# Triton-AI/Triton-Racer-Sim

Measured on AMD Instinct MI355X. Metric: env-steps/s (whole node) at N envs x 120x160 RGB, higher is better.
Workload: dtype f32 state / f64 nearest-point / u8 image; 1 GPU; 1024 envs/GPU x 1 GPU, bicycle physics + L1 nearest point + 120x160 RGB pinhole rasteriser = BASELINE configs[2], generated_track 1185 pts, synthetic controls seed 0x5EED, auto-reset; envs_total=1024, envs_per_gpu=1024, img_h=120, img_w=160, depth=False, steps_per_launch=1, step_mode=resident worker (posted steps), prewarm_steps=8400, launcher=self

## Files before the change

### triton-racer-sim_amd/csrc/trsim_post.hpp

```cpp
#pragma once

#include <algorithm>
#include <chrono>
#include <cstddef>
#include <cstdint>
#include <cstring>

#include "trsim_plan.hpp"

namespace trsim {

constexpr int kSlots = 8;

struct WEntry {
    uint64_t seq_lo;
    const float* steer; const float* thr; const float* brk;
    const uint8_t* reset;
    uint32_t synth, pad0;
    uint64_t seq;
    uint64_t pad1;
};
static_assert(sizeof(WEntry) == 64, "one entry per 64-B line");
constexpr int kTagLo = 0, kTagHi = 6;
static_assert(offsetof(WEntry, seq_lo) == 8 * kTagLo && offsetof(WEntry, seq) == 8 * kTagHi && offsetof(WEntry, reset) == 32, "tag placement");

struct Mailbox {
    alignas(64) uint64_t close;
    uint64_t posted;
    alignas(64) uint64_t exited;
    uint64_t consumed;
    uint64_t error;
    uint64_t started;
    alignas(64) uint64_t done[kSlots];
    alignas(64) WEntry ring[kSlots];
};

constexpr unsigned long long kExitNormal = 1ull, kExitNotCoresident = 2ull;
constexpr unsigned long long kCloseLeave = 1ull, kCloseCancel = 2ull;
constexpr unsigned kRetryMs0 = 100;

enum GiveUp : unsigned { kGiveUpPost = 1, kGiveUpCamRing = 2, kGiveUpPhysics = 3, kGiveUpForward = 4, kGiveUpBarrier = 5, kGiveUpInjected = 7, kGiveUpLdsBase = 9 };
constexpr const char* kGiveUpText[10] = {"", "waiting for a post", "camera ring back-pressure", "waiting for the physics team", "forwarding the last arrivals",
                                         "team barrier of the dynamic-brightness batch", "", "abort injected by trs_resident_debug_abort (test hook)", "",
                                         "dynamic LDS segment not at offset 0"};
inline const char* give_up_text(unsigned code) { return code < 10 ? kGiveUpText[code] : "?"; }

inline uint64_t host_load(const uint64_t* p) { return __atomic_load_n(p, __ATOMIC_ACQUIRE); }
inline void host_store(uint64_t* p, uint64_t v) { __atomic_store_n(p, v, __ATOMIC_RELEASE); }

struct PostLedger {
    using Clock = std::chrono::steady_clock;
    bool enabled = false;
    bool running = false;
    bool launched = false;
    bool fell_back = false;
    bool broken = false;
    uint64_t base = 0;
    uint64_t seen_done = 0;
    unsigned retry_ms = kRetryMs0;
    Clock::time_point t_fallback{};

    void restart(uint64_t step) { base = seen_done = step; }
    void absorb(uint64_t step) { launched = false; restart(step); }
    void note_launch(uint64_t step) { launched = true; restart(step); }
    void observe(uint64_t count) { seen_done = std::max(seen_done, count); }
    bool orphans(uint64_t posted, uint64_t step) const { return posted > seen_done && posted == step; }
    bool must_wait(uint64_t s) const { return s >= base + kSlots; }
    void worker_launched() { running = true; }
    void worker_ended() { running = false; }
    void worker_had_the_gpu() { retry_ms = kRetryMs0; }
    void gave_up() { broken = true; }
    void clear_fault() { broken = false; }
    void fall_back(Clock::time_point now) { enabled = false; fell_back = true; t_fallback = now; }
    bool retry_due(Clock::time_point now) const { return !enabled && fell_back && !broken && now - t_fallback >= std::chrono::milliseconds(retry_ms); }
    bool select(uint64_t step) { retry_ms = kRetryMs0; return turn_on(step); }
    bool reselect(uint64_t step) { retry_ms = std::min(retry_ms * 2u, 2000u); launched = false; return turn_on(step); }
    void deselect() { enabled = false; }
private:
// ... 33 lines not shown
```

### triton-racer-sim_amd/csrc/trsim_resident.hip

```cpp
#include <hip/hip_runtime.h>

#include <algorithm>
#include <array>
#include <atomic>
#include <chrono>
#include <cstdint>
#include <cstdlib>
#include <cstring>
#include <mutex>
#include <string>
#include <utility>

#include "../../include/trsim.h"
#include "../../include/trsim_spec.h"
#include "trsim_device.hpp"
#include "trsim_env.hpp"
#include "trsim_internal.hpp"
#include "trsim_post.hpp"

namespace trsim {

struct DevCtl {
    alignas(64) unsigned long long word;
    alignas(64) WEntry ring[kSlots];
// ... 21 lines not shown
#ifndef TRS_RESIDENT_DIAG
#define TRS_RESIDENT_DIAG 0
#endif
constexpr int kDiag = TRS_RESIDENT_DIAG;

constexpr unsigned kDefaultLifeUs = 50000;
#ifndef TRS_PHYS_PRIO_MAX_ENVS
#define TRS_PHYS_PRIO_MAX_ENVS 1
#endif

struct Resident {
    PostLedger led;
    PinnedBuf<Mailbox> mb;
    DevBuf<DevCtl> dc;
    hipStream_t sC = nullptr;
    uint64_t gen_start = 0; Variant gen_variant = 0;
    bool dc_ready = false; uint64_t dc_ready_for = 0;
    std::chrono::steady_clock::time_point t_launch{};
    unsigned idle_us = 2000;
    unsigned life_us = kDefaultLifeUs;
    PinnedBuf<> hctl;
    int lds_bytes = 0, lds_off_ctl = 0, lds_off_dyn = 0, lds_off_hill = 0;
    long long pw_capacity_envs = 0;
    int pw_capacity_lds = -1;
};

}

namespace {

using namespace trsim;
using u64 = unsigned long long;

constexpr u64 kExitBit = 1ull << 63, kAbortBit = 1ull << 62, kCountMask = kAbortBit - 1;
constexpr int kFellBack = trsim::kResidentFellBack;

constexpr int kMaxDevices = 64;
struct DeviceSlot { std::recursive_mutex mu; trs_env* owner = nullptr; };
DeviceSlot g_dev[kMaxDevices];
struct DevLock {
    std::unique_lock<std::recursive_mutex> lk;
    explicit DevLock(const trs_env* e) : lk(g_dev[(unsigned)e->device % kMaxDevices].mu) {}
};
inline DeviceSlot& slot_of(const trs_env* e) { return g_dev[(unsigned)e->device % kMaxDevices]; }

__device__ __forceinline__ u64 sys_load64(const void* p) { return __hip_atomic_load((const u64*)p, __ATOMIC_RELAXED, __HIP_MEMORY_SCOPE_SYSTEM); }
__device__ __forceinline__ unsigned sys_load32(const void* p) { return __hip_atomic_load((const unsigned*)p, __ATOMIC_RELAXED, __HIP_MEMORY_SCOPE_SYSTEM); }
__device__ __forceinline__ void sys_store64(void* p, u64 v) { __hip_atomic_store((u64*)p, v, __ATOMIC_RELAXED, __HIP_MEMORY_SCOPE_SYSTEM); }
__device__ __forceinline__ u64 agent_load64(const void* p) { return __hip_atomic_load((const u64*)p, __ATOMIC_RELAXED, __HIP_MEMORY_SCOPE_AGENT); }
__device__ __forceinline__ void agent_store64(void* p, u64 v) { __hip_atomic_store((u64*)p, v, __ATOMIC_RELAXED, __HIP_MEMORY_SCOPE_AGENT); }
__device__ __forceinline__ u64 lds_load64(const u64* p) { return __hip_atomic_load(p, __ATOMIC_RELAXED, __HIP_MEMORY_SCOPE_WORKGROUP); }
__device__ __forceinline__ void lds_store64(u64* p, u64 v) { __hip_atomic_store(p, v, __ATOMIC_RELAXED, __HIP_MEMORY_SCOPE_WORKGROUP); }
__device__ __forceinline__ int lds_load32(const int* p) { return __hip_atomic_load(p, __ATOMIC_RELAXED, __HIP_MEMORY_SCOPE_WORKGROUP); }
__device__ __forceinline__ void lds_store32(int* p, int v) { __hip_atomic_store(p, v, __ATOMIC_RELAXED, __HIP_MEMORY_SCOPE_WORKGROUP); }
__device__ __forceinline__ void drain_vmem() { asm volatile("s_waitcnt vmcnt(0)" ::: "memory"); }
__device__ __forceinline__ void drain_lds() { asm volatile("s_waitcnt lgkmcnt(0)" ::: "memory"); }

__device__ __forceinline__ void wait_vmcnt_le(int n)
{
    switch (__builtin_amdgcn_readfirstlane(n < 0 ? 0 : (n > 63 ? 63 : n))) {
#define W(i) case i: asm volatile("s_waitcnt vmcnt(" #i ")" ::: "memory"); break;
    W(0) W(1) W(2) W(3) W(4) W(5) W(6) W(7) W(8) W(9) W(10) W(11) W(12) W(13) W(14) W(15) W(16) W(17) W(18) W(19) W(20) W(21) W(22) W(23) W(24) W(25) W(26) W(27) W(28) W(29) W(30) W(31) W(32) W(33) W(34) W(35) W(36) W(37) W(38) W(39) W(40) W(41) W(42) W(43) W(44) W(45) W(46) W(47) W(48) W(49) W(50) W(51) W(52) W(53) W(54) W(55) W(56) W(57) W(58) W(59) W(60) W(61) W(62) W(63)
#undef W
    }
}

template <typename T>
__device__ __forceinline__ T sys_load_val(const T* p)
{
    return __hip_atomic_load((const __attribute__((address_space(1))) T*)(uintptr_t)p, __ATOMIC_RELAXED, __HIP_MEMORY_SCOPE_SYSTEM);
}

struct WLds {
    u64* word;
    u64* fwd;
    int* arrive;
    int* pprog;
    int* rread;
    float* slot;
    float* lst;
};

__device__ __forceinline__ WLds wlds_of(unsigned char* base, int epw)
{
    WLds l;
    l.word = reinterpret_cast<u64*>(base);
    l.fwd = reinterpret_cast<u64*>(base + 8);
    l.arrive = reinterpret_cast<int*>(base + 16);
    l.pprog = reinterpret_cast<int*>(base + 64);
    l.rread = l.pprog + epw;
    l.slot = reinterpret_cast<float*>(base + wlds_slot_off(epw));
    l.lst = l.slot + (size_t)kCamDepth * epw * kSlotWords;
    return l;
}

__device__ __forceinline__ void worker_abort(const WParams& wp, const WLds& l, unsigned code)
{
    sys_store64(&wp.mb->error, ((u64)code << 32) | (u64)blockIdx.x);
    __hip_atomic_fetch_or(&wp.dc->word, kAbortBit, __ATOMIC_RELAXED, __HIP_MEMORY_SCOPE_AGENT);
    __hip_atomic_fetch_or(l.word, kAbortBit, __ATOMIC_RELAXED, __HIP_MEMORY_SCOPE_WORKGROUP);
}

struct Leader { u64 known, t_last, t_start; };

__device__ __forceinline__ u64 lane_u64(u64 v, int k)
{
    return ((u64)(unsigned)__builtin_amdgcn_readlane((int)(v >> 32), k) << 32) | (u64)(unsigned)__builtin_amdgcn_readlane((int)v, k);
}

__device__ __forceinline__ int dispatcher_take(const WParams& wp, const WLds& l, Leader& L, int lane, bool& close_req)
{
    const u64 v = sys_load64(reinterpret_cast<const u64*>(&wp.mb->ring[0]) + lane);
    const u64 c = sys_load64(&wp.mb->close);
    close_req = c != 0ull;
    int fresh = 0;
    for (; fresh < kSlots; ++fresh) {
        const int slot = (int)((L.known + (u64)fresh) & (kSlots - 1));
        const int hi = slot * 8 + kTagHi, lo = slot * 8 + kTagLo;
        const u64 tag = ((u64)(unsigned)__shfl((int)(v >> 32), hi, 64) << 32) | (u64)(unsigned)__shfl((int)v, hi, 64);
        const u64 tag_lo = ((u64)(unsigned)__shfl((int)(v >> 32), lo, 64) << 32) | (u64)(unsigned)__shfl((int)v, lo, 64);
        if (tag != L.known + (u64)fresh + 1 || tag_lo != tag) break;
    }
    if (fresh == 0) return 0;
    const int rel = (int)(((u64)(lane >> 3) - L.known) & (kSlots - 1));
    if (rel < fresh) agent_store64(reinterpret_cast<u64*>(&wp.dc->ring[0]) + lane, v);
    drain_vmem();
    L.known += (u64)fresh;
    if (lane == 0) {
        __hip_atomic_fetch_max(&wp.dc->word, L.known, __ATOMIC_RELAXED, __HIP_MEMORY_SCOPE_AGENT);
        __hip_atomic_fetch_max(l.word, L.known, __ATOMIC_RELAXED, __HIP_MEMORY_SCOPE_WORKGROUP);
    }
    return fresh;
}

__device__ __forceinline__ void dispatcher_publish_exit(const WParams& wp, const WLds& l, u64 count, int lane)
{
    if (lane == 0) {
        const u64 w = count | kExitBit;
        const u64 old_g = __hip_atomic_fetch_max(&wp.dc->word, w, __ATOMIC_RELAXED, __HIP_MEMORY_SCOPE_AGENT);
        if (old_g & kAbortBit) __hip_atomic_fetch_or(&wp.dc->word, kAbortBit, __ATOMIC_RELAXED, __HIP_MEMORY_SCOPE_AGENT);
        const u64 old_l = __hip_atomic_fetch_max(l.word, w, __ATOMIC_RELAXED, __HIP_MEMORY_SCOPE_WORKGROUP);
        if ((old_l | old_g) & kAbortBit) __hip_atomic_fetch_or(l.word, kAbortBit, __ATOMIC_RELAXED, __HIP_MEMORY_SCOPE_WORKGROUP);
    }
    drain_vmem();
}

__device__ __forceinline__ void worker_checkin(const WParams& wp)
{
    __hip_atomic_fetch_add(&wp.dc->checkin[0], 1u, __ATOMIC_RELAXED, __HIP_MEMORY_SCOPE_AGENT);
}

constexpr unsigned kGo = 1u, kNoGo = 2u;

__device__ __forceinline__ unsigned decision_load(const WParams& wp) { return __hip_atomic_load(&wp.dc->decision[0], __ATOMIC_RELAXED, __HIP_MEMORY_SCOPE_AGENT); }

__device__ __forceinline__ unsigned decision_close(const WParams& wp, unsigned want, int lane, bool& won)
{
    unsigned seen = 0u;
    if (lane == 0) {
        unsigned expected = 0u;
        const bool ok = __hip_atomic_compare_exchange_strong(&wp.dc->decision[0], &expected, want, __ATOMIC_RELAXED, __ATOMIC_RELAXED, __HIP_MEMORY_SCOPE_AGENT);
        seen = ok ? (want | 0x100u) : expected;
    }
    seen = (unsigned)__builtin_amdgcn_readfirstlane((int)seen);
    won = (seen & 0x100u) != 0u;
    return seen & 0xffu;
}

__device__ __forceinline__ void leave_not_coresident(const WParams& wp, const WLds& l, int lane, bool won)
{
    if (won) {
        if (lane == 0) sys_store64(&wp.mb->consumed, wp.start);
        drain_vmem();
        if (lane == 0) sys_store64(&wp.mb->exited, kExitNotCoresident);
    }
    dispatcher_publish_exit(wp, l, wp.start, lane);
}

__device__ __forceinline__ int dispatcher_checkin(const WParams& wp, const WLds& l, int lane)
{
    const u64 t0 = (u64)wall_clock64();
    bool cancel = sys_load64(&wp.mb->close) == kCloseCancel, won = false;
    for (unsigned spins = 0; !cancel; ++spins) {
        if (decision_load(wp) == kNoGo) { leave_not_coresident(wp, l, lane, false); return 0; }
        if (__hip_atomic_load(&wp.dc->checkin[0], __ATOMIC_RELAXED, __HIP_MEMORY_SCOPE_AGENT) >= (unsigned)wp.n_blocks) {
            if (decision_close(wp, kGo, lane, won) != kGo) { leave_not_coresident(wp, l, lane, false); return 0; }
            if (lane == 0) sys_store64(&wp.mb->started, 1ull);
            return 1;
        }
        if (agent_load64(&wp.dc->word) & kAbortBit) {
            if (lane == 0) __hip_atomic_fetch_or(l.word, kAbortBit, __ATOMIC_RELAXED, __HIP_MEMORY_SCOPE_WORKGROUP);
            return 0;
        }
        if ((u64)wall_clock64() - t0 > wp.checkin_ticks) break;
        if ((spins & 63u) == 63u) cancel = sys_load64(&wp.mb->close) == kCloseCancel;
        __builtin_amdgcn_s_sleep(4);
    }
    const unsigned d = decision_close(wp, kNoGo, lane, won);
    if (d == kGo) { if (lane == 0) sys_store64(&wp.mb->started, 1ull); return 1; }
    leave_not_coresident(wp, l, lane, won);
    return 0;
}

__device__ __forceinline__ int leader_wait_decision(const WParams& wp, const WLds& l, int lane)
{
    const u64 t0 = (u64)wall_clock64();
    for (;;) {
        unsigned d = decision_load(wp);
        if (d == 0u && (u64)wall_clock64() - t0 > 2ull * wp.checkin_ticks) {
            bool won = false;
            d = decision_close(wp, kNoGo, lane, won);
            if (d == kNoGo) { leave_not_coresident(wp, l, lane, won); return 0; }
        }
        if (d == kGo) return 1;
        if (d == kNoGo) { leave_not_coresident(wp, l, lane, false); return 0; }
        if (agent_load64(&wp.dc->word) & kAbortBit) {
            if (lane == 0) __hip_atomic_fetch_or(l.word, kAbortBit, __ATOMIC_RELAXED, __HIP_MEMORY_SCOPE_WORKGROUP);
            return 0;
        }
        __builtin_amdgcn_s_sleep(8);
    }
}

__device__ __forceinline__ void dispatcher_run(const WParams& wp, const WLds& l, int lane)
{
    if (!dispatcher_checkin(wp, l, lane)) return;
    Leader L{wp.start, (u64)wall_clock64(), (u64)wall_clock64()};
    for (;;) {
        if ((lds_load64(l.word) | agent_load64(&wp.dc->word)) & kAbortBit) {
            if (lane == 0) __hip_atomic_fetch_or(l.word, kAbortBit, __ATOMIC_RELAXED, __HIP_MEMORY_SCOPE_WORKGROUP);
            return;
        }
        const u64 now = (u64)wall_clock64();
        bool close_req = false;
        const int fresh = dispatcher_take(wp, l, L, lane, close_req);
        const bool busy = (u64)lds_load64(l.fwd) < L.known;
        if (fresh || busy) L.t_last = now;
        const bool leave = (!fresh && (close_req || now - L.t_last > wp.idle_ticks)) || now - L.t_start > wp.life_ticks;
        if (!leave) { if (!fresh) __builtin_amdgcn_s_sleep(4); continue; }
        if (lane == 0) sys_store64(&wp.mb->exited, kExitNormal);
        drain_vmem();
        (void)dispatcher_take(wp, l, L, lane, close_req);
        if (lane == 0) sys_store64(&wp.mb->consumed, L.known);
        dispatcher_publish_exit(wp, l, L.known, lane);
        return;
    }
}

__device__ __forceinline__ void raster_arrive(const WLds& l, u64 s, int lane)
{
    if (lane == 0) __hip_atomic_fetch_add(&l.arrive[s & (kSlots - 1)], 1, __ATOMIC_RELAXED, __HIP_MEMORY_SCOPE_WORKGROUP);
}

__device__ __forceinline__ void forward_arrivals(const WParams& wp, const WLds& l, u64& fwd, int lane, int want = kRasterThreads / 64)
{
    const int slot = (int)(fwd & (kSlots - 1));
    if (lds_load32(&l.arrive[slot]) != want) return;
    if (lane == 0) {
        lds_store32(&l.arrive[slot], 0);
        const int shard = (int)(blockIdx.x & 7u), nshards = min(8, wp.n_blocks);
        const unsigned members = (unsigned)((wp.n_blocks - shard + 7) / 8);
        const unsigned uses = (unsigned)((fwd - wp.start) / (u64)kSlots) + 1u;
        unsigned* a = &wp.dc->arrive[slot][shard][0];
        if (__hip_atomic_fetch_add(a, 1u, __ATOMIC_RELAXED, __HIP_MEMORY_SCOPE_AGENT) == members * uses - 1u) {
            unsigned* t = &wp.dc->top[slot][0];
            if (__hip_atomic_fetch_add(t, 1u, __ATOMIC_RELAXED, __HIP_MEMORY_SCOPE_AGENT) == (unsigned)nshards * uses - 1u)
                sys_store64(&wp.mb->done[slot], fwd + 1);
        }
    }
    fwd += 1;
    if (lane == 0) lds_store64(l.fwd, fwd);
}

struct Duties { bool leader, forwarder; u64 fwd; int want = kRasterThreads / 64; };

__device__ __forceinline__ int wait_posted(const WParams& wp, const WLds& l, Duties& D, u64 s, int lane)
{
    u64 t0 = 0;
    for (unsigned spins = 0;; ++spins) {
        if (D.forwarder) forward_arrivals(wp, l, D.fwd, lane, D.want);
        const u64 w = lds_load64(l.word);
        if (w & kAbortBit) return 0;
        if ((w & kCountMask) > s) return 1;
        if (w & kExitBit) return 0;
        if (D.leader) {
            const u64 g = agent_load64(&wp.dc->word);
            if (g != w) { if (lane == 0) lds_store64(l.word, g); drain_lds(); continue; }
        }
        __builtin_amdgcn_s_sleep(4);
        if ((spins & 255u) == 255u) {
            const u64 now = (u64)wall_clock64();
            if (t0 == 0) t0 = now;
            else if (now - t0 > wp.safety_ticks) { worker_abort(wp, l, kGiveUpPost); return 0; }
        }
    }
}

__device__ __forceinline__ int wait_lds_ge(const WParams& wp, const WLds& l, Duties* D, const int* ctr, int want, unsigned code, int lane)
{
    u64 t0 = 0;
    for (unsigned spins = 0;; ++spins) {
        if (lds_load32(ctr) >= want) return 1;
        if (D && D->forwarder) forward_arrivals(wp, l, D->fwd, lane, D->want);
        __builtin_amdgcn_s_sleep(1);
        if ((spins & 1023u) == 1023u) {
            if (lds_load64(l.word) & kAbortBit) return 0;
            const u64 now = (u64)wall_clock64();
            if (t0 == 0) t0 = now;
            else if (now - t0 > wp.safety_ticks) { worker_abort(wp, l, code); return 0; }
        }
    }
}

template <bool DEPTH, bool DYN, bool HILLS = false, bool LENS = false, bool LIGHT = false>
__global__ __launch_bounds__(kBlock) void trs_worker_kernel(const WParams wp)
{
    const int tid = threadIdx.x, lane = tid & 63, wave = tid >> 6;
    const bool raster_team = tid < kRasterThreads;
    const RParams& p = wp.ra;
    const PParams& P = wp.ph;
    const int epw = p.envs_per_wg;
    const WLds l = wlds_of(smem + wp.lds_off_ctl, epw);
    const int e_begin = blockIdx.x * epw;
    const int n_loc = min(e_begin + epw, p.n_envs) - e_begin;
    const int pw = wave - kRasterThreads / 64;
    if ((unsigned)(uintptr_t)smem != 0u) {
        if (tid == 0) {
            atomicAdd(&p.stats[2], 1ull);
            sys_store64(p.fault, 1ull);
            sys_store64(&wp.mb->error, ((u64)kGiveUpLdsBase << 32) | (u64)blockIdx.x);
            __hip_atomic_fetch_or(&wp.dc->word, kAbortBit, __ATOMIC_RELAXED, __HIP_MEMORY_SCOPE_AGENT);
            if (blockIdx.x == 0) { sys_store64(&wp.mb->consumed, wp.start); sys_store64(&wp.mb->exited, 1ull); }
        }
        return;
    }
    if (raster_team) stage_lds_dma(p.blob, p.blob_bytes, 0u, wave, kRasterThreads / 64, lane);
    else stage_lds_dma(P.blob, P.blob_bytes, (unsigned)wp.lds_off_phys, pw, kPhysWaves, lane);
    if (LENS && raster_team) lens_stage_palette(p, (unsigned)wp.lds_off_hill, wave, lane);
    if (tid == 0) { lds_store64(l.word, wp.start); lds_store64(l.fwd, wp.start); }
    if (tid < kSlots) l.arrive[tid] = 0;
    for (int j = tid; j < 2 * epw; j += kBlock) l.pprog[j] = 0;
    int* const hbar = reinterpret_cast<int*>(smem + wp.lds_off_hill + hill_batch(p.H) * hill_table_bytes(p.H));
    if (HILLS && tid == 0) *hbar = 0;
    const int lds_off_light = worker_lds_light(wp.lds_off_hill, p.H, variant_bits(DEPTH, DYN, HILLS, LENS, LIGHT));
    float* const lring = reinterpret_cast<float*>(smem + lds_off_light);
    const unsigned lds_off_lpal = (unsigned)lds_off_light + (unsigned)(kCamDepth * epw * 32);
    const float* const light_g = LIGHT ? hill_block(p)->light : nullptr;
    const int lfilt = LIGHT ? hill_block(p)->filt : 0;
    if constexpr (DYN) {
        if (tid < 32) reinterpret_cast<int*>(smem + wp.fp.lds_off + kDynBatch * p.H * 16)[tid] = 0;
        dyn_stage_tables(smem, wp.fp, p.H, tid, kBlock, reinterpret_cast<const uint32_t*>(p.blob + p.off_pal));
    }
    if (!raster_team)
        for (int j = pw; j < n_loc; j += kPhysWaves) {
            EnvRegs st;
            env_load(P, e_begin + j, st);
            const float lr = coherent_load(&P.last_return[e_begin + j]);
            if (lane == 0) {
                float* q = l.lst + (size_t)j * 16;
                q[0] = st.x; q[1] = st.y; q[2] = st.z; q[3] = st.yaw; q[4] = st.v; q[5] = st.sf; q[6] = st.epr;
                q[7] = __int_as_float(st.seg); q[8] = __int_as_float(st.epl); q[9] = __int_as_float(st.done); q[10] = __int_as_float(st.pend);
                q[11] = lr;
            }
        }
    asm volatile("s_waitcnt vmcnt(0) lgkmcnt(0)" ::: "memory");
    __syncthreads();
    if (tid == 0) worker_checkin(wp);

    if (!raster_team) {
        const int first = blockIdx.x == 0 ? 1 : 0, nphys = kPhysWaves - first;
        if (pw < first) { dispatcher_run(wp, l, lane); return; }
        Duties D{blockIdx.x != 0 && pw == 0, pw == kPhysWaves - 1, wp.start};
        if (D.leader && !leader_wait_decision(wp, l, lane)) return;
        const unsigned char* const lphys = smem + wp.lds_off_phys;
        u64 s = wp.start;
        for (;; ++s) {
            const int r = (int)(s - wp.start);
            if (!wait_posted(wp, l, D, s, lane)) break;
            const u64* en = reinterpret_cast<const u64*>(&wp.dc->ring[s & (kSlots - 1)]);
            const u64 ev = lane < 6 ? agent_load64(en + lane) : 0ull;
            const float* const c_st = reinterpret_cast<const float*>(lane_u64(ev, 1));
            const float* const c_th = reinterpret_cast<const float*>(lane_u64(ev, 2));
            const float* const c_br = reinterpret_cast<const float*>(lane_u64(ev, 3));
            const uint8_t* const c_rs = reinterpret_cast<const uint8_t*>(lane_u64(ev, 4));
            const int synth = (int)(unsigned)lane_u64(ev, 5);
            for (int j = pw - first; j < n_loc; j += nphys) {
                const int e = e_begin + j;
                if (r >= kCamDepth && !wait_lds_ge(wp, l, &D, &l.rread[j], (r - kCamDepth + 1) * (kRasterThreads / 64), kGiveUpCamRing, lane)) return;
                float steer = 0.f, thr = 0.f, brk = 0.f;
                uint8_t rin = 0;
                if (!synth) {
                    steer = sys_load_val(&c_st[e]); thr = sys_load_val(&c_th[e]);
                    if (c_br) brk = sys_load_val(&c_br[e]);
                    if (c_rs) rin = sys_load_val(&c_rs[e]);
                }
                float* const q = l.lst + (size_t)j * 16;
                EnvRegs st;
                st.x = q[0]; st.y = q[1]; st.z = q[2]; st.yaw = q[3]; st.v = q[4]; st.sf = q[5]; st.epr = q[6];
                st.seg = __float_as_int(q[7]); st.epl = __float_as_int(q[8]); st.done = __float_as_int(q[9]); st.pend = __float_as_int(q[10]);
                st.speed = 0.f; st.cte = 0.f;
                float lr = q[11];
                const float epr_before = st.epr;
                StepOut o;
                if (n_loc <= TRS_PHYS_PRIO_MAX_ENVS) __builtin_amdgcn_s_setprio(3);
                env_advance<true, false>(P, lphys, e, st, (uint32_t)s, synth, steer, thr, brk, rin, lane, o, HILLS ? hill_block(p) : nullptr);
                if (n_loc <= TRS_PHYS_PRIO_MAX_ENVS) __builtin_amdgcn_s_setprio(0);
                if (o.do_reset) lr = epr_before;
                if constexpr (LIGHT) {
                    const float lv = lane < 8 ? sys_load_val(&light_g[(size_t)e * 8 + lane]) : 0.f;
                    if (lane < 8) lring[((size_t)(r & (kCamDepth - 1)) * epw + j) * 8 + lane] = lv;
                }
                if (lane == 0) {
                    q[0] = st.x; q[1] = st.y; q[2] = st.z; q[3] = st.yaw; q[4] = st.v; q[5] = st.sf; q[6] = st.epr;
                    q[7] = __int_as_float(st.seg); q[8] = __int_as_float(st.epl); q[9] = __int_as_float(st.done); q[10] = __int_as_float(st.pend);
                    q[11] = lr;
                    float* const sl = l.slot + ((size_t)(r & (kCamDepth - 1)) * epw + j) * kSlotWords;
                    *reinterpret_cast<float4*>(sl) = o.cam;
                    sl[4] = st.x; sl[5] = st.y; sl[6] = st.z; sl[7] = st.yaw; sl[8] = st.v; sl[9] = st.speed; sl[10] = st.cte;
                    sl[11] = __int_as_float(st.seg); sl[12] = st.epr; sl[13] = __int_as_float(st.epl); sl[14] = st.sf; sl[15] = lr;
                    sl[16] = __int_as_float(st.done);
                    if constexpr (HILLS) sl[17] = o.pitch;
                    if (o.is_done) atomicAdd(&P.stats[0], 1ull);
                    if (o.do_reset) atomicAdd(&P.stats[1], 1ull);
                    drain_lds();
                    lds_store32(&l.pprog[j], r + 1);
                }
            }
        }
        if (D.forwarder) {
            u64 t0 = 0;
            for (unsigned spins = 0; D.fwd < s; ++spins) {
                forward_arrivals(wp, l, D.fwd, lane);
                if (lds_load64(l.word) & kAbortBit) break;
                __builtin_amdgcn_s_sleep(2);
                if ((spins & 1023u) == 1023u) {
                    const u64 now = (u64)wall_clock64();
                    if (t0 == 0) t0 = now;
                    else if (now - t0 > wp.safety_ticks) { worker_abort(wp, l, kGiveUpForward); break; }
                }
            }
        }
        return;
    }

    const RasterThread rth = raster_thread(p, smem, tid);
    trsim::LensBlock lb{};
    LensCacheWorker<DEPTH> lcache;
    if constexpr (LENS) {
        lb = *lens_block(p);
        lens_cache_load(p, rth, lb, lcache);
    }
    int nu = 0, ng = 0;
    for (int v = rth.vstart; v < p.uni_rows; v += p.rows_per_pass) ++nu;
    for (int v = rth.vground; v < p.H; v += p.rows_per_pass) ++ng;
#pragma unroll
    for (int off = 32; off >= 1; off >>= 1) { nu = max(nu, __shfl_xor(nu, off, 64)); ng = max(ng, __shfl_xor(ng, off, 64)); }
    nu *= DEPTH ? 2 : 1; ng *= DEPTH ? 2 : 1;
    int own = 0;
    for (int j = wave; j < n_loc; j += kRasterThreads / 64) ++own;
    const int nuni = nu * n_loc, nstep = (nu + ng) * n_loc + 2 * own;
    constexpr bool kSkipUniform = !DYN && !HILLS && !LIGHT && !LENS;
    const int lag = worker_lag(nstep, nuni, kSkipUniform);
    unsigned char* optr = nullptr;
    {
        unsigned char* const tab[14] = {(unsigned char*)P.x, (unsigned char*)P.y, (unsigned char*)P.z, (unsigned char*)P.yaw, (unsigned char*)P.v,
                                        (unsigned char*)P.speed, (unsigned char*)P.cte, (unsigned char*)P.seg_idx, (unsigned char*)P.ep_return,
                                        (unsigned char*)P.ep_len, (unsigned char*)P.steer_filt, (unsigned char*)P.last_return,
                                        (unsigned char*)P.done, (unsigned char*)P.pending};
#pragma unroll
        for (int k = 0; k < 14; ++k) optr = lane == k ? tab[k] : optr;
    }
    Duties none{false, false, 0};
    u64 owed = wp.start;
    const bool probe = (kDiag & 4) && blockIdx.x == 7 && wave == 0;
    auto now_clk = [&]() -> u64 { u64 t; asm volatile("s_memtime %0\n\ts_waitcnt lgkmcnt(0)" : "=s"(t) :: "memory"); return t; };
    u64 t_post = 0, t_pose = 0, t_vm = 0, t_all = 0, t_mark = probe ? now_clk() : 0;
    for (u64 s = wp.start;; ++s) {
        const int r = (int)(s - wp.start);
        if (owed < s && (lds_load64(l.word) & kCountMask) <= s) {
            drain_vmem();
            for (; owed < s; ++owed) raster_arrive(l, owed, lane);
        }
        const u64 tp0 = probe ? now_clk() : 0;
        if (!wait_posted(wp, l, none, s, lane)) {
            drain_vmem();
            for (; owed < s; ++owed) raster_arrive(l, owed, lane);
            if (probe && lane == 0) {
                t_all = now_clk() - t_mark;
                atomicAdd(&p.stats[40], t_post); atomicAdd(&p.stats[41], t_pose); atomicAdd(&p.stats[42], t_vm); atomicAdd(&p.stats[43], t_all);
                atomicAdd(&p.stats[44], (u64)r);
            }
            return;
        }
        if (probe) t_post += now_clk() - tp0;
        uint8_t* const img = (s & 1ull) ? wp.img1 : wp.img0;
        float* const dep = (s & 1ull) ? wp.dep1 : wp.dep0;
        const u64 ahead = (lds_load64(l.word) & kCountMask) - 1 - s;
        const u64 keep = ahead + 1 < (u64)lag ? ahead + 1 : (u64)lag;
        if constexpr (DYN) {
            while (s - owed >= keep) {
                wait_vmcnt_le((int)(s - owed - 1) * nstep);
                raster_arrive(l, owed++, lane);
            }
            const int nbatch = (n_loc + kDynBatch - 1) / kDynBatch;
            for (int b0 = 0; b0 < n_loc; b0 += kDynBatch) {
                float4 cams[kDynBatch];
                unsigned tel = 0; int mine_j = -1;
#pragma unroll
                for (int bi = 0; bi < kDynBatch; ++bi) {
                    const int j = b0 + bi;
                    cams[bi] = make_float4(0.f, 0.f, 0.f, 1.f);
                    if (j < n_loc) {
                        if (!wait_lds_ge(wp, l, nullptr, &l.pprog[j], r + 1, kGiveUpPhysics, lane)) return;
                        const float* const sl = l.slot + ((size_t)(r & (kCamDepth - 1)) * epw + j) * kSlotWords;
                        cams[bi] = *reinterpret_cast<const float4*>(sl);
                        if ((j % (kRasterThreads / 64)) == wave) { mine_j = j; tel = __float_as_uint(sl[4 + min(lane, 12)]); }
                        asm volatile("s_waitcnt lgkmcnt(0)" :: "v"(cams[bi].x), "v"(cams[bi].y), "v"(cams[bi].z), "v"(cams[bi].w), "v"(tel) : "memory");
                        if (!LIGHT && lane == 0) __hip_atomic_fetch_add(&l.rread[j], 1, __ATOMIC_RELAXED, __HIP_MEMORY_SCOPE_WORKGROUP);
                    }
                }
                u64 t0_bar = 0;
                auto bail = [&](bool first) -> bool {
                    if (lds_load64(l.word) & kAbortBit) return true;
                    const u64 now = (u64)wall_clock64();
                    if (first) { t0_bar = now; return false; }
                    if (now - t0_bar > wp.safety_ticks) { worker_abort(wp, l, kGiveUpBarrier); return true; }
                    return false;
                };
                if (!raster_dyn_batch<DEPTH, LIGHT>(p, wp.fp, rth, smem, cams, min(kDynBatch, n_loc - b0), img, dep, e_begin + b0, r * nbatch + b0 / kDynBatch, tid, lane, bail,
                                                   LIGHT ? lring + ((size_t)(r & (kCamDepth - 1)) * epw + b0) * 8 : nullptr, lds_off_lpal)) return;
// ... 64 lines not shown
                const float* const sl = l.slot + ((size_t)(r & (kCamDepth - 1)) * epw + j) * kSlotWords;
                const float4 cam = *reinterpret_cast<const float4*>(sl);
                const bool mine = (j % (kRasterThreads / 64)) == wave;
                unsigned tel = 0;
                if (mine) tel = __float_as_uint(sl[4 + min(lane, 12)]);
                RasterThread rl = rth;
                rl.pal_off = light_wave_palette(p, lds_off_lpal, lring + ((size_t)(r & (kCamDepth - 1)) * epw + j) * 8, lfilt, wave, lane);
                asm volatile("s_waitcnt lgkmcnt(0)" :: "v"(cam.x), "v"(cam.y), "v"(cam.z), "v"(cam.w), "v"(tel) : "memory");
                if (lane == 0) __hip_atomic_fetch_add(&l.rread[j], 1, __ATOMIC_RELAXED, __HIP_MEMORY_SCOPE_WORKGROUP);
                raster_uniform_rows<DEPTH>(p, rl, fd);
                if (j == 0)
                    while (s - owed >= keep) {
                        wait_vmcnt_le((int)(s - owed - 1) * nstep + nu);
                        raster_arrive(l, owed++, lane);
                    }
                raster_ground_rows<DEPTH>(p, rl, fd, cam);
                if (mine && !(kDiag & 2)) {
                    const size_t e = (size_t)(e_begin + j);
                    if (lane < 12) __hip_atomic_store((__attribute__((address_space(1))) unsigned*)(uintptr_t)optr + e, tel, __ATOMIC_RELAXED, __HIP_MEMORY_SCOPE_SYSTEM);
                    else if (lane < 14) __hip_atomic_store((__attribute__((address_space(1))) unsigned char*)(uintptr_t)optr + e, (unsigned char)(lane == 12 ? tel : 0u), __ATOMIC_RELAXED, __HIP_MEMORY_SCOPE_SYSTEM);
                }
            }
            continue;
        }
        const bool skipu = kSkipUniform && worker_skips_uniform(wp.uni_mask, wp.start, s);
        const bool sweep = ahead == 0 && !skipu;
        if (sweep)
            for (int j = 0; j < n_loc; ++j) raster_uniform_rows<DEPTH>(p, rth, frame_desc<DEPTH>(p, img, dep, e_begin + j));
        for (int j = 0; j < n_loc; ++j) {
            const FrameDesc fd = frame_desc<DEPTH>(p, img, dep, e_begin + j);
            if (!sweep && !skipu) raster_uniform_rows<DEPTH>(p, rth, fd);
            if (j == 0)
                while (s - owed >= keep) {
                    const u64 tv0 = probe ? now_clk() : 0;
                    if (!(kDiag & 1))
                        wait_vmcnt_le(kSkipUniform ? worker_wait_count(wp.uni_mask, wp.start, owed, s, nstep, nuni, skipu ? 0 : (sweep ? nuni : nu))
                                                   : (int)(s - owed - 1) * nstep + (sweep ? nuni : nu));
                    if (probe) t_vm += now_clk() - tv0;
                    raster_arrive(l, owed++, lane);
                }
            const u64 tq0 = probe ? now_clk() : 0;
            if (!wait_lds_ge(wp, l, nullptr, &l.pprog[j], r + 1, kGiveUpPhysics, lane)) return;
            if (probe) t_pose += now_clk() - tq0;
            const float* const sl = l.slot + ((size_t)(r & (kCamDepth - 1)) * epw + j) * kSlotWords;
            const float4 cam = *reinterpret_cast<const float4*>(sl);
            const bool mine = (j % (kRasterThreads / 64)) == wave;
            unsigned tel = 0;
            if (mine) tel = __float_as_uint(sl[4 + min(lane, 12)]);
            asm volatile("s_waitcnt lgkmcnt(0)" :: "v"(cam.x), "v"(cam.y), "v"(cam.z), "v"(cam.w), "v"(tel) : "memory");
            if (lane == 0) __hip_atomic_fetch_add(&l.rread[j], 1, __ATOMIC_RELAXED, __HIP_MEMORY_SCOPE_WORKGROUP);
            if constexpr (LENS) raster_lens_frame(p, rth, lb, lcache, (unsigned)wp.lds_off_hill, fd, cam);
            else raster_ground_rows<DEPTH>(p, rth, fd, cam);
            if (mine && !(kDiag & 2)) {
                const size_t e = (size_t)(e_begin + j);
                if (lane < 12) __hip_atomic_store((__attribute__((address_space(1))) unsigned*)(uintptr_t)optr + e, tel, __ATOMIC_RELAXED, __HIP_MEMORY_SCOPE_SYSTEM);
                else if (lane < 14) __hip_atomic_store((__attribute__((address_space(1))) unsigned char*)(uintptr_t)optr + e, (unsigned char)(lane == 12 ? tel : 0u), __ATOMIC_RELAXED, __HIP_MEMORY_SCOPE_SYSTEM);
            }
        }
    }
}

using WorkerKernel = void (*)(WParams);
template <Variant V> WorkerKernel worker_kernel_of()
{
    if constexpr (variant_built(V)) return &trs_worker_kernel<(V & kVDepth) != 0, (V & kVDyn) != 0, (V & kVHills) != 0, (V & kVLens) != 0, (V & kVLight) != 0>;
    else return nullptr;
}
template <Variant... V> std::array<WorkerKernel, kVariants> worker_kernel_table(std::integer_sequence<Variant, V...>) { return {worker_kernel_of<V>()...}; }
const std::array<WorkerKernel, kVariants> kWorkerKernels = worker_kernel_table(std::make_integer_sequence<Variant, kVariants>{});

constexpr int kPwEnvs = 4;
constexpr int kPwBlock = 64 * (kPwEnvs + 2);

__global__ __launch_bounds__(kPwBlock) void trs_physics_worker_kernel(const WParams wp)
{
    const int tid = threadIdx.x, lane = tid & 63, wave = tid >> 6;
    const PParams& P = wp.ph;
    const WLds l = wlds_of(smem + wp.lds_off_ctl, kPwEnvs);
    const int e_begin = blockIdx.x * kPwEnvs;
    const int n_loc = min(e_begin + kPwEnvs, P.n_envs) - e_begin;
    if ((unsigned)(uintptr_t)smem != 0u) {
        if (tid == 0) {
            atomicAdd(&P.stats[2], 1ull);
            sys_store64(P.fault, 1ull);
            sys_store64(&wp.mb->error, ((u64)kGiveUpLdsBase << 32) | (u64)blockIdx.x);
            __hip_atomic_fetch_or(&wp.dc->word, kAbortBit, __ATOMIC_RELAXED, __HIP_MEMORY_SCOPE_AGENT);
            if (blockIdx.x == 0) { sys_store64(&wp.mb->consumed, wp.start); sys_store64(&wp.mb->exited, 1ull); }
        }
        return;
    }
    stage_lds_dma(P.blob, P.blob_bytes, 0u, wave, kPwBlock / 64, lane);
    if (tid == 0) { lds_store64(l.word, wp.start); lds_store64(l.fwd, wp.start); }
    if (tid < kSlots) l.arrive[tid] = 0;
    asm volatile("s_waitcnt vmcnt(0) lgkmcnt(0)" ::: "memory");
    __syncthreads();
    if (tid == 0) worker_checkin(wp);

    if (wave == kPwEnvs + 1) {
        if (blockIdx.x == 0) dispatcher_run(wp, l, lane);
        return;
    }
    if (wave == kPwEnvs) {
        Duties D{blockIdx.x != 0, true, wp.start, n_loc};
        if (D.leader && !leader_wait_decision(wp, l, lane)) return;
        u64 s = wp.start;
        while (wait_posted(wp, l, D, s, lane)) ++s;
        const u64 w = lds_load64(l.word);
        if (w & kAbortBit) return;
        const u64 last = w & kCountMask;
        u64 t0 = 0;
        for (unsigned spins = 0; D.fwd < last; ++spins) {
            forward_arrivals(wp, l, D.fwd, lane, n_loc);
            if (lds_load64(l.word) & kAbortBit) break;
            __builtin_amdgcn_s_sleep(2);
            if ((spins & 1023u) == 1023u) {
                const u64 now = (u64)wall_clock64();
                if (t0 == 0) t0 = now;
                else if (now - t0 > wp.safety_ticks) { worker_abort(wp, l, kGiveUpForward); break; }
            }
        }
        return;
    }
    if (wave >= n_loc) return;

    const int e = e_begin + wave;
    EnvRegs st;
    env_load(P, e, st);
    float lr = coherent_load(&P.last_return[e]);
    unsigned char* optr = nullptr;
    {
        unsigned char* const tab[14] = {(unsigned char*)P.x, (unsigned char*)P.y, (unsigned char*)P.z, (unsigned char*)P.yaw, (unsigned char*)P.v,
                                        (unsigned char*)P.speed, (unsigned char*)P.cte, (unsigned char*)P.seg_idx, (unsigned char*)P.ep_return,
                                        (unsigned char*)P.ep_len, (unsigned char*)P.steer_filt, (unsigned char*)P.last_return,
                                        (unsigned char*)P.done, (unsigned char*)P.pending};
#pragma unroll
        for (int k = 0; k < 14; ++k) optr = lane == k ? tab[k] : optr;
    }
    Duties none{false, false, 0};
    u64 owed = wp.start;
    struct Ctl { float steer, thr, brk; uint8_t rin; int synth; };
    auto entry_load = [&](u64 s) -> u64 {
        const u64* en = reinterpret_cast<const u64*>(&wp.dc->ring[s & (kSlots - 1)]);
        return lane < 6 ? agent_load64(en + lane) : 0ull;
    };
    auto ctl_load = [&](u64 ev) -> Ctl {
        const float* const c_st = reinterpret_cast<const float*>(lane_u64(ev, 1));
        const float* const c_th = reinterpret_cast<const float*>(lane_u64(ev, 2));
        const float* const c_br = reinterpret_cast<const float*>(lane_u64(ev, 3));
        const uint8_t* const c_rs = reinterpret_cast<const uint8_t*>(lane_u64(ev, 4));
        Ctl in{0.f, 0.f, 0.f, 0, (int)(unsigned)lane_u64(ev, 5)};
        asm volatile("" :: "s"(c_st), "s"(c_th), "s"(in.synth) : "memory");
        if (!in.synth) {
            in.steer = sys_load_val(&c_st[e]); in.thr = sys_load_val(&c_th[e]);
            if (c_br) in.brk = sys_load_val(&c_br[e]);
            if (c_rs) in.rin = sys_load_val(&c_rs[e]);
        }
        return in;
    };
    bool have_ctl = false, have_ent = false;
    Ctl nxt{};
    u64 ent_next = 0ull;
    u64 clean_below = wp.start;
    for (u64 s = wp.start;; ++s) {
        if (owed < s && (lds_load64(l.word) & kCountMask) <= s) {
            drain_vmem();
            for (; owed < s; ++owed) raster_arrive(l, owed, lane);
            clean_below = s;
        }
        Ctl in;
        if (have_ctl) {
            in = nxt;
        } else {
            if (!wait_posted(wp, l, none, s, lane)) {
                drain_vmem();
                for (; owed < s; ++owed) raster_arrive(l, owed, lane);
                return;
            }
            in = ctl_load(entry_load(s));
            drain_vmem();
            clean_below = s;
        }
        const u64 count = lds_load64(l.word) & kCountMask;
        have_ctl = count > s + 1;
        if (have_ctl) {
            const bool was_prefetched = have_ent;
            nxt = ctl_load(was_prefetched ? ent_next : entry_load(s + 1));
            const u64 c = was_prefetched ? s - 1 : s;
            clean_below = c > clean_below ? c : clean_below;
        }
        have_ent = have_ctl && count > s + 2;
        if (have_ent) ent_next = entry_load(s + 2);
        for (; owed < clean_below; ++owed) raster_arrive(l, owed, lane);
        const float epr_before = st.epr;
        StepOut o;
        env_advance<true, false, true>(P, smem, e, st, (uint32_t)s, in.synth, in.steer, in.thr, in.brk, in.rin, lane, o);
        if (o.do_reset) lr = epr_before;
        if (lane == 0) {
            if (o.is_done) atomicAdd(&P.stats[0], 1ull);
            if (o.do_reset) atomicAdd(&P.stats[1], 1ull);
        }
        unsigned tel = 0;
        {
            const unsigned vals[13] = {__float_as_uint(st.x), __float_as_uint(st.y), __float_as_uint(st.z), __float_as_uint(st.yaw), __float_as_uint(st.v),
                                       __float_as_uint(st.speed), __float_as_uint(st.cte), (unsigned)st.seg, __float_as_uint(st.epr), (unsigned)st.epl,
                                       __float_as_uint(st.sf), __float_as_uint(lr), (unsigned)st.done};
#pragma unroll
            for (int k = 0; k < 13; ++k) tel = lane == k ? vals[k] : tel;
        }
        if (lane < 12) __hip_atomic_store((__attribute__((address_space(1))) unsigned*)(uintptr_t)optr + e, tel, __ATOMIC_RELAXED, __HIP_MEMORY_SCOPE_SYSTEM);
        else if (lane < 14) __hip_atomic_store((__attribute__((address_space(1))) unsigned char*)(uintptr_t)optr + e, (unsigned char)(lane == 12 ? tel : 0u), __ATOMIC_RELAXED, __HIP_MEMORY_SCOPE_SYSTEM);
    }
}

__global__ void trs_worker_init_kernel(DevCtl* dc, u64 start)
{
    unsigned* w = reinterpret_cast<unsigned*>(dc);
    for (int i = threadIdx.x; i < (int)(sizeof(DevCtl) / 4); i += blockDim.x) w[i] = 0u;
    __syncthreads();
    if (threadIdx.x == 0) agent_store64(&dc->word, start);
}


int worker_fits(trs_env* e)
{
    Resident* R = e->res;
    if (!e->cfg.render) {
        R->lds_off_ctl = (e->lds_p + 15) & ~15;
        R->lds_bytes = (int)(R->lds_off_ctl + wlds_bytes(kPwEnvs) + 16);
        if (R->lds_bytes > 160 * 1024) return trs_internal_fail(TRS_ERR_LIMIT, "track image too large for the resident physics worker");
        if (R->pw_capacity_lds != R->lds_bytes) {
            int per_cu = 0;
            HIPCHK(hipOccupancyMaxActiveBlocksPerMultiprocessor(&per_cu, reinterpret_cast<const void*>(trs_physics_worker_kernel), kPwBlock, (size_t)R->lds_bytes));
            R->pw_capacity_envs = (long long)per_cu * (long long)std::max(e->cu_count, 1) * kPwEnvs;
            R->pw_capacity_lds = R->lds_bytes;
        }
        const long long capacity = R->pw_capacity_envs / kPwEnvs;
        const long long grid = ((long long)e->n + kPwEnvs - 1) / kPwEnvs;
        if (capacity > 0 && grid > capacity)
            return trs_internal_fail(TRS_ERR_LIMIT, "resident mode: " + std::to_string(e->n) + " physics-only envs need " + std::to_string(grid) +
                                                        " co-resident workgroups, this GPU holds " + std::to_string(capacity) + " (" + std::to_string(capacity * kPwEnvs) +
                                                        " envs): use TRS_STEP_LAUNCH with several steps per launch for shards of this size");
        return TRS_OK;
    }
    const WorkerLds L = worker_lds_layout(e->lds_step, e->pp.envs_per_wg, e->H, e->W, variant_of(e));
    R->lds_off_ctl = L.ctl; R->lds_off_dyn = L.dyn; R->lds_off_hill = L.hill; R->lds_bytes = L.total;
    if (R->lds_bytes > 160 * 1024)
        return trs_internal_fail(TRS_ERR_LIMIT, e->scene.hilly ? "the resident worker's LDS state and the per-env row tables of a track with elevation do not fit beside this track's tables: use TRS_STEP_LAUNCH"
                                                : e->scene.lens_on ? "the resident worker's LDS state and the lens camera's palette do not fit beside this track's tables: use TRS_STEP_LAUNCH"
                                                : e->scene.light_on ? "the resident worker's LDS state and the lit palettes of scene lighting do not fit beside this track's tables: use TRS_STEP_LAUNCH"
                                                            : "too many envs per workgroup for the resident worker's LDS state");
    return TRS_OK;
}
// ... 357 lines not shown
```

Before: 125.9 million env-steps/s.

## Pack run-length of identical posts into step word to skip ring entry reloads

The dispatcher now detects when consecutive posted ring entries carry the same control pointers and packs a run length into the low bits of the shared step counter word. Physics waves in the render worker reuse the entry they already hold instead of reloading the 64-B ring line from agent-scope memory each step when the run covers the current step. This is meant to cut a global load from each step's critical path, but it adds shuffles and ballots in the dispatcher and narrows the counter by four bits. Diagnostic timing probes gated by kDiag are added as well.

```diff
diff --git a/triton-racer-sim_amd/csrc/trsim_post.hpp b/triton-racer-sim_amd/csrc/trsim_post.hpp
--- a/triton-racer-sim_amd/csrc/trsim_post.hpp
+++ b/triton-racer-sim_amd/csrc/trsim_post.hpp
@@ -44,6 +44,20 @@
                                          "team barrier of the dynamic-brightness batch", "", "abort injected by trs_resident_debug_abort (test hook)", "",
                                          "dynamic LDS segment not at offset 0"};
 inline const char* give_up_text(unsigned code) { return code < 10 ? kGiveUpText[code] : "?"; }
+
+constexpr unsigned long long kExitBit = 1ull << 63, kAbortBit = 1ull << 62;
+constexpr int kRunBits = 4;
+constexpr unsigned long long kRunMax = (1ull << kRunBits) - 1;
+constexpr unsigned long long kCountMax = (kAbortBit >> kRunBits) - 1;
+constexpr unsigned long long word_pack(unsigned long long count, unsigned long long run) { return (count << kRunBits) | (run < kRunMax ? run : kRunMax); }
+constexpr unsigned long long word_count(unsigned long long w) { return (w & (kAbortBit - 1)) >> kRunBits; }
+constexpr unsigned long long word_run(unsigned long long w) { return w & kRunMax; }
+constexpr unsigned long long run_note(unsigned long long same_from, unsigned long long step, bool payload_equal_to_previous) { return payload_equal_to_previous ? same_from : step; }
+constexpr unsigned long long run_of(unsigned long long same_from, unsigned long long count) { return count - same_from < kRunMax ? count - same_from : kRunMax; }
+constexpr bool entry_reusable(unsigned long long held_step, unsigned long long s, unsigned long long count, unsigned long long run)
+{
+    return s > 0 && held_step == s - 1 && count > s && s - 1 + run >= count;
+}
 
 inline uint64_t host_load(const uint64_t* p) { return __atomic_load_n(p, __ATOMIC_ACQUIRE); }
 inline void host_store(uint64_t* p, uint64_t v) { __atomic_store_n(p, v, __ATOMIC_RELEASE); }
diff --git a/triton-racer-sim_amd/csrc/trsim_resident.hip b/triton-racer-sim_amd/csrc/trsim_resident.hip
--- a/triton-racer-sim_amd/csrc/trsim_resident.hip
+++ b/triton-racer-sim_amd/csrc/trsim_resident.hip
@@ -77,7 +77,6 @@
 using namespace trsim;
 using u64 = unsigned long long;
 
-constexpr u64 kExitBit = 1ull << 63, kAbortBit = 1ull << 62, kCountMask = kAbortBit - 1;
 constexpr int kFellBack = trsim::kResidentFellBack;
 
 constexpr int kMaxDevices = 64;
@@ -100,6 +99,11 @@
 __device__ __forceinline__ void lds_store32(int* p, int v) { __hip_atomic_store(p, v, __ATOMIC_RELAXED, __HIP_MEMORY_SCOPE_WORKGROUP); }
 __device__ __forceinline__ void drain_vmem() { asm volatile("s_waitcnt vmcnt(0)" ::: "memory"); }
 __device__ __forceinline__ void drain_lds() { asm volatile("s_waitcnt lgkmcnt(0)" ::: "memory"); }
+__device__ __forceinline__ u64 uniform_u64(u64 v)
+{
+    return ((u64)(unsigned)__builtin_amdgcn_readfirstlane((int)(v >> 32)) << 32) | (u64)(unsigned)__builtin_amdgcn_readfirstlane((int)v);
+}
+__device__ __forceinline__ u64 probe_clk() { u64 t; asm volatile("s_memtime %0\n\ts_waitcnt lgkmcnt(0)" : "=s"(t) :: "memory"); return t; }
 
 __device__ __forceinline__ void wait_vmcnt_le(int n)
 {
@@ -146,7 +150,7 @@
     __hip_atomic_fetch_or(l.word, kAbortBit, __ATOMIC_RELAXED, __HIP_MEMORY_SCOPE_WORKGROUP);
 }
 
-struct Leader { u64 known, t_last, t_start; };
+struct Leader { u64 known, t_last, t_start, same_from, prev; bool have_prev; };
 
 __device__ __forceinline__ u64 lane_u64(u64 v, int k)
 {
@@ -169,19 +173,28 @@
     if (fresh == 0) return 0;
     const int rel = (int)(((u64)(lane >> 3) - L.known) & (kSlots - 1));
     if (rel < fresh) agent_store64(reinterpret_cast<u64*>(&wp.dc->ring[0]) + lane, v);
+    for (int f = 0; f < fresh; ++f) {
+        const int src = (int)((L.known + (u64)f) & (kSlots - 1)) * 8 + (lane & 7);
+        const u64 cur = ((u64)(unsigned)__shfl((int)(v >> 32), src, 64) << 32) | (u64)(unsigned)__shfl((int)v, src, 64);
+        const bool differs = (lane & 7) >= 1 && (lane & 7) <= 5 && cur != L.prev;
+        const bool equal = L.have_prev && __ballot(differs) == 0ull;
+        L.same_from = run_note(L.same_from, L.known + (u64)f, equal);
+        L.prev = cur; L.have_prev = true;
+    }
     drain_vmem();
     L.known += (u64)fresh;
     if (lane == 0) {
-        __hip_atomic_fetch_max(&wp.dc->word, L.known, __ATOMIC_RELAXED, __HIP_MEMORY_SCOPE_AGENT);
-        __hip_atomic_fetch_max(l.word, L.known, __ATOMIC_RELAXED, __HIP_MEMORY_SCOPE_WORKGROUP);
+        const u64 w = word_pack(L.known, run_of(L.same_from, L.known));
+        __hip_atomic_fetch_max(&wp.dc->word, w, __ATOMIC_RELAXED, __HIP_MEMORY_SCOPE_AGENT);
+        __hip_atomic_fetch_max(l.word, w, __ATOMIC_RELAXED, __HIP_MEMORY_SCOPE_WORKGROUP);
     }
     return fresh;
 }
 
-__device__ __forceinline__ void dispatcher_publish_exit(const WParams& wp, const WLds& l, u64 count, int lane)
+__device__ __forceinline__ void dispatcher_publish_exit(const WParams& wp, const WLds& l, u64 count, u64 run, int lane)
 {
     if (lane == 0) {
-        const u64 w = count | kExitBit;
+        const u64 w = word_pack(count, run) | kExitBit;
         const u64 old_g = __hip_atomic_fetch_max(&wp.dc->word, w, __ATOMIC_RELAXED, __HIP_MEMORY_SCOPE_AGENT);
         if (old_g & kAbortBit) __hip_atomic_fetch_or(&wp.dc->word, kAbortBit, __ATOMIC_RELAXED, __HIP_MEMORY_SCOPE_AGENT);
         const u64 old_l = __hip_atomic_fetch_max(l.word, w, __ATOMIC_RELAXED, __HIP_MEMORY_SCOPE_WORKGROUP);
@@ -219,7 +232,7 @@
         drain_vmem();
         if (lane == 0) sys_store64(&wp.mb->exited, kExitNotCoresident);
     }
-    dispatcher_publish_exit(wp, l, wp.start, lane);
+    dispatcher_publish_exit(wp, l, wp.start, 0, lane);
 }
 
 __device__ __forceinline__ int dispatcher_checkin(const WParams& wp, const WLds& l, int lane)
@@ -270,7 +283,7 @@
 __device__ __forceinline__ void dispatcher_run(const WParams& wp, const WLds& l, int lane)
 {
     if (!dispatcher_checkin(wp, l, lane)) return;
-    Leader L{wp.start, (u64)wall_clock64(), (u64)wall_clock64()};
+    Leader L{wp.start, (u64)wall_clock64(), (u64)wall_clock64(), wp.start, 0ull, false};
     for (;;) {
         if ((lds_load64(l.word) | agent_load64(&wp.dc->word)) & kAbortBit) {
             if (lane == 0) __hip_atomic_fetch_or(l.word, kAbortBit, __ATOMIC_RELAXED, __HIP_MEMORY_SCOPE_WORKGROUP);
@@ -287,7 +300,7 @@
         drain_vmem();
         (void)dispatcher_take(wp, l, L, lane, close_req);
         if (lane == 0) sys_store64(&wp.mb->consumed, L.known);
-        dispatcher_publish_exit(wp, l, L.known, lane);
+        dispatcher_publish_exit(wp, l, L.known, run_of(L.same_from, L.known), lane);
         return;
     }
 }
@@ -319,14 +332,14 @@
 
 struct Duties { bool leader, forwarder; u64 fwd; int want = kRasterThreads / 64; };
 
-__device__ __forceinline__ int wait_posted(const WParams& wp, const WLds& l, Duties& D, u64 s, int lane)
+__device__ __forceinline__ int wait_posted(const WParams& wp, const WLds& l, Duties& D, u64 s, int lane, u64* seen = nullptr)
 {
     u64 t0 = 0;
     for (unsigned spins = 0;; ++spins) {
         if (D.forwarder) forward_arrivals(wp, l, D.fwd, lane, D.want);
         const u64 w = lds_load64(l.word);
         if (w & kAbortBit) return 0;
-        if ((w & kCountMask) > s) return 1;
+        if (word_count(w) > s) { if (seen) *seen = w; return 1; }
         if (w & kExitBit) return 0;
         if (D.leader) {
             const u64 g = agent_load64(&wp.dc->word);
@@ -382,7 +395,7 @@
     if (raster_team) stage_lds_dma(p.blob, p.blob_bytes, 0u, wave, kRasterThreads / 64, lane);
     else stage_lds_dma(P.blob, P.blob_bytes, (unsigned)wp.lds_off_phys, pw, kPhysWaves, lane);
     if (LENS && raster_team) lens_stage_palette(p, (unsigned)wp.lds_off_hill, wave, lane);
-    if (tid == 0) { lds_store64(l.word, wp.start); lds_store64(l.fwd, wp.start); }
+    if (tid == 0) { lds_store64(l.word, word_pack(wp.start, 0)); lds_store64(l.fwd, wp.start); }
     if (tid < kSlots) l.arrive[tid] = 0;
     for (int j = tid; j < 2 * epw; j += kBlock) l.pprog[j] = 0;
     int* const hbar = reinterpret_cast<int*>(smem + wp.lds_off_hill + hill_batch(p.H) * hill_table_bytes(p.H));
@@ -418,20 +431,38 @@
         Duties D{blockIdx.x != 0 && pw == 0, pw == kPhysWaves - 1, wp.start};
         if (D.leader && !leader_wait_decision(wp, l, lane)) return;
         const unsigned char* const lphys = smem + wp.lds_off_phys;
+        const bool pprobe = (kDiag & 8) && pw == 1 && (blockIdx.x == 7 || blockIdx.x == 0);
+        u64 q_post = 0, q_entry = 0, q_ring = 0, q_adv = 0, q_hand = 0, q_loads = 0;
         u64 s = wp.start;
+        constexpr bool kReuseEntry = !DEPTH && !LIGHT;
+        u64 ev = 0ull, held = 0ull;
         for (;; ++s) {
             const int r = (int)(s - wp.start);
-            if (!wait_posted(wp, l, D, s, lane)) break;
-            const u64* en = reinterpret_cast<const u64*>(&wp.dc->ring[s & (kSlots - 1)]);
-            const u64 ev = lane < 6 ? agent_load64(en + lane) : 0ull;
+            u64 seen = 0ull;
+            const u64 tq0 = pprobe ? probe_clk() : 0;
+            if (!wait_posted(wp, l, D, s, lane, &seen)) break;
+            const u64 tq1 = pprobe ? probe_clk() : 0;
+            const u64 w = uniform_u64(seen);
+            if (r == 0 || !kReuseEntry || (kDiag & 16) || !entry_reusable(held, s, word_count(w), word_run(w))) {
+                const u64* en = reinterpret_cast<const u64*>(&wp.dc->ring[s & (kSlots - 1)]);
+                ev = lane < 6 ? agent_load64(en + lane) : 0ull;
+                if (pprobe) ++q_loads;
+            }
+            held = s;
             const float* const c_st = reinterpret_cast<const float*>(lane_u64(ev, 1));
             const float* const c_th = reinterpret_cast<const float*>(lane_u64(ev, 2));
             const float* const c_br = reinterpret_cast<const float*>(lane_u64(ev, 3));
             const uint8_t* const c_rs = reinterpret_cast<const uint8_t*>(lane_u64(ev, 4));
             const int synth = (int)(unsigned)lane_u64(ev, 5);
+            if (pprobe) {
+                asm volatile("" :: "s"(c_st), "s"(c_th), "s"(c_br), "s"(c_rs), "s"(synth) : "memory");
+                q_post += tq1 - tq0; q_entry += probe_clk() - tq1;
+            }
             for (int j = pw - first; j < n_loc; j += nphys) {
                 const int e = e_begin + j;
+                const u64 tq2 = pprobe ? probe_clk() : 0;
                 if (r >= kCamDepth && !wait_lds_ge(wp, l, &D, &l.rread[j], (r - kCamDepth + 1) * (kRasterThreads / 64), kGiveUpCamRing, lane)) return;
+                const u64 tq3 = pprobe ? probe_clk() : 0;
                 float steer = 0.f, thr = 0.f, brk = 0.f;
                 uint8_t rin = 0;
                 if (!synth) {
@@ -450,6 +481,8 @@
                 if (n_loc <= TRS_PHYS_PRIO_MAX_ENVS) __builtin_amdgcn_s_setprio(3);
                 env_advance<true, false>(P, lphys, e, st, (uint32_t)s, synth, steer, thr, brk, rin, lane, o, HILLS ? hill_block(p) : nullptr);
                 if (n_loc <= TRS_PHYS_PRIO_MAX_ENVS) __builtin_amdgcn_s_setprio(0);
+                u64 tq4 = 0;
+                if (pprobe) { asm volatile("" :: "v"(o.cam.x), "v"(o.cam.w), "v"(st.x), "v"(st.epr) : "memory"); tq4 = probe_clk(); }
                 if (o.do_reset) lr = epr_before;
                 if constexpr (LIGHT) {
                     const float lv = lane < 8 ? sys_load_val(&light_g[(size_t)e * 8 + lane]) : 0.f;
@@ -470,7 +503,13 @@
                     drain_lds();
                     lds_store32(&l.pprog[j], r + 1);
                 }
-            }
+                if (pprobe) { drain_lds(); q_ring += tq3 - tq2; q_adv += tq4 - tq3; q_hand += probe_clk() - tq4; }
+            }
+        }
+        if (pprobe && lane == 0) {
+            unsigned long long* const out = p.stats + (blockIdx.x == 7 ? 8 : 16);
+            atomicAdd(&out[0], q_post); atomicAdd(&out[1], q_entry); atomicAdd(&out[2], q_ring); atomicAdd(&out[3], q_adv); atomicAdd(&out[4], q_hand);
+            atomicAdd(&out[5], q_loads); atomicAdd(&out[6], s - wp.start);
         }
         if (D.forwarder) {
             u64 t0 = 0;
@@ -518,29 +557,28 @@
     Duties none{false, false, 0};
     u64 owed = wp.start;
     const bool probe = (kDiag & 4) && blockIdx.x == 7 && wave == 0;
-    auto now_clk = [&]() -> u64 { u64 t; asm volatile("s_memtime %0\n\ts_waitcnt lgkmcnt(0)" : "=s"(t) :: "memory"); return t; };
-    u64 t_post = 0, t_pose = 0, t_vm = 0, t_all = 0, t_mark = probe ? now_clk() : 0;
+    u64 t_post = 0, t_pose = 0, t_vm = 0, t_all = 0, t_mark = probe ? probe_clk() : 0;
     for (u64 s = wp.start;; ++s) {
         const int r = (int)(s - wp.start);
-        if (owed < s && (lds_load64(l.word) & kCountMask) <= s) {
+        if (owed < s && word_count(lds_load64(l.word)) <= s) {
             drain_vmem();
             for (; owed < s; ++owed) raster_arrive(l, owed, lane);
         }
-        const u64 tp0 = probe ? now_clk() : 0;
+        const u64 tp0 = probe ? probe_clk() : 0;
         if (!wait_posted(wp, l, none, s, lane)) {
             drain_vmem();
             for (; owed < s; ++owed) raster_arrive(l, owed, lane);
             if (probe && lane == 0) {
-                t_all = now_clk() - t_mark;
+                t_all = probe_clk() - t_mark;
                 atomicAdd(&p.stats[40], t_post); atomicAdd(&p.stats[41], t_pose); atomicAdd(&p.stats[42], t_vm); atomicAdd(&p.stats[43], t_all);
                 atomicAdd(&p.stats[44], (u64)r);
             }
             return;
         }
-        if (probe) t_post += now_clk() - tp0;
+        if (probe) t_post += probe_clk() - tp0;
         uint8_t* const img = (s & 1ull) ? wp.img1 : wp.img0;
         float* const dep = (s & 1ull) ? wp.dep1 : wp.dep0;
-        const u64 ahead = (lds_load64(l.word) & kCountMask) - 1 - s;
+        const u64 ahead = word_count(lds_load64(l.word)) - 1 - s;
         const u64 keep = ahead + 1 < (u64)lag ? ahead + 1 : (u64)lag;
         if constexpr (DYN) {
             while (s - owed >= keep) {
@@ -671,16 +709,16 @@
             if (!sweep && !skipu) raster_uniform_rows<DEPTH>(p, rth, fd);
             if (j == 0)
                 while (s - owed >= keep) {
-                    const u64 tv0 = probe ? now_clk() : 0;
+                    const u64 tv0 = probe ? probe_clk() : 0;
                     if (!(kDiag & 1))
                         wait_vmcnt_le(kSkipUniform ? worker_wait_count(wp.uni_mask, wp.start, owed, s, nstep, nuni, skipu ? 0 : (sweep ? nuni : nu))
                                                    : (int)(s - owed - 1) * nstep + (sweep ? nuni : nu));
-                    if (probe) t_vm += now_clk() - tv0;
+                    if (probe) t_vm += probe_clk() - tv0;
                     raster_arrive(l, owed++, lane);
                 }
-            const u64 tq0 = probe ? now_clk() : 0;
+            const u64 tq0 = probe ? probe_clk() : 0;
             if (!wait_lds_ge(wp, l, nullptr, &l.pprog[j], r + 1, kGiveUpPhysics, lane)) return;
-            if (probe) t_pose += now_clk() - tq0;
+            if (probe) t_pose += probe_clk() - tq0;
             const float* const sl = l.slot + ((size_t)(r & (kCamDepth - 1)) * epw + j) * kSlotWords;
             const float4 cam = *reinterpret_cast<const float4*>(sl);
             const bool mine = (j % (kRasterThreads / 64)) == wave;
@@ -729,7 +767,7 @@
         return;
     }
     stage_lds_dma(P.blob, P.blob_bytes, 0u, wave, kPwBlock / 64, lane);
-    if (tid == 0) { lds_store64(l.word, wp.start); lds_store64(l.fwd, wp.start); }
+    if (tid == 0) { lds_store64(l.word, word_pack(wp.start, 0)); lds_store64(l.fwd, wp.start); }
     if (tid < kSlots) l.arrive[tid] = 0;
     asm volatile("s_waitcnt vmcnt(0) lgkmcnt(0)" ::: "memory");
     __syncthreads();
@@ -746,7 +784,7 @@
         while (wait_posted(wp, l, D, s, lane)) ++s;
         const u64 w = lds_load64(l.word);
         if (w & kAbortBit) return;
-        const u64 last = w & kCountMask;
+        const u64 last = word_count(w);
         u64 t0 = 0;
         for (unsigned spins = 0; D.fwd < last; ++spins) {
             forward_arrivals(wp, l, D.fwd, lane, n_loc);
@@ -801,7 +839,7 @@
     u64 ent_next = 0ull;
     u64 clean_below = wp.start;
     for (u64 s = wp.start;; ++s) {
-        if (owed < s && (lds_load64(l.word) & kCountMask) <= s) {
+        if (owed < s && word_count(lds_load64(l.word)) <= s) {
             drain_vmem();
             for (; owed < s; ++owed) raster_arrive(l, owed, lane);
             clean_below = s;
@@ -819,7 +857,7 @@
             drain_vmem();
             clean_below = s;
         }
-        const u64 count = lds_load64(l.word) & kCountMask;
+        const u64 count = word_count(lds_load64(l.word));
         have_ctl = count > s + 1;
         if (have_ctl) {
             const bool was_prefetched = have_ent;
@@ -856,7 +894,7 @@
     unsigned* w = reinterpret_cast<unsigned*>(dc);
     for (int i = threadIdx.x; i < (int)(sizeof(DevCtl) / 4); i += blockDim.x) w[i] = 0u;
     __syncthreads();
-    if (threadIdx.x == 0) agent_store64(&dc->word, start);
+    if (threadIdx.x == 0) agent_store64(&dc->word, word_pack(start, 0));
 }
 
 
```

Result: faster. 127.5 million env-steps/s, median of 6 (+1.3%).
